# PathologyFoundation/plip

Measured on AMD Instinct MI355X. Metric: image+text pairs embedded/sec at 224px bs=256, higher is better.
Workload: dtype bf16; 1 GPU; full dual encoder (image tower + text tower + L2 normalise + logits_per_image), ViT-B/32, bs=256 pairs per GPU, 224px, 77 tokens, bf16 MFMA / fp32 accumulate (BASELINE.json configs[2]); the first 8 of the 12 text blocks on f16 MFMA operands (plipmi_config.text_f16_layers, the engine default); arch=ViT-B/32, per_gpu_batch=256, global_batch=256, parallelism=dp1, collective=none, streams=2, device=gfx950:sramecc+:xnack-:AMD Radeon Graphics

## Files before the change

### plip_amd/_lib.py

```python
from __future__ import annotations

import ctypes as C
import os
from typing import Optional

import torch

_HERE = os.path.dirname(os.path.abspath(__file__))
LIB_PATH = os.path.join(_HERE, "csrc", "libplipmi.so")

F32, BF16, F16 = 0, 1, 2
FLAG_SEPARATE_LAYERNORM, FLAG_DENSE_LAST_BLOCK, FLAG_PACK_CAPTIONS, FLAG_VALU_ATTENTION, FLAG_TEXT_TOWER_F16 = 1, 2, 4, 8, 16
FLAG_VISION_GELU, FLAG_TEXT_GELU = 32, 64
VISION, TEXT = 0, 1


class Config(C.Structure):
    _fields_ = [(n, C.c_int32) for n in (
        "struct_size", "image_size", "patch_size", "v_width", "v_layers", "v_heads", "v_mlp", "vocab_size",
        "context_length", "t_width", "t_layers", "t_heads", "t_mlp", "projection_dim")] + [
        ("layer_norm_eps", C.c_float), ("compute_dtype", C.c_int32), ("max_batch", C.c_int32), ("flags", C.c_int32),
        ("graph_batch", C.c_int32), ("text_f16_layers", C.c_int32), ("pass_batch", C.c_int32)]


_LAYER_FIELDS = ("ln1_w", "ln1_b", "q_w", "q_b", "k_w", "k_b", "v_w", "v_b", "o_w", "o_b",
                 "ln2_w", "ln2_b", "fc1_w", "fc1_b", "fc2_w", "fc2_b")


class LayerWeights(C.Structure):
    _fields_ = [(n, C.c_void_p) for n in _LAYER_FIELDS]


class Weights(C.Structure):
    _fields_ = [
        ("v_class_embedding", C.c_void_p), ("v_patch_weight", C.c_void_p), ("v_pos_embedding", C.c_void_p),
        ("v_pre_ln_w", C.c_void_p), ("v_pre_ln_b", C.c_void_p), ("v_post_ln_w", C.c_void_p),
        ("v_post_ln_b", C.c_void_p), ("visual_projection", C.c_void_p), ("v_layers", C.POINTER(LayerWeights)),
        ("t_token_embedding", C.c_void_p), ("t_pos_embedding", C.c_void_p), ("t_final_ln_w", C.c_void_p),
        ("t_final_ln_b", C.c_void_p), ("text_projection", C.c_void_p), ("t_layers", C.POINTER(LayerWeights)),
    ]


WEIGHT_KEYS = {
    "v_class_embedding": "vision_model.embeddings.class_embedding", "v_patch_weight": "vision_model.embeddings.patch_embedding.weight",
    "v_pos_embedding": "vision_model.embeddings.position_embedding.weight", "v_pre_ln_w": "vision_model.pre_layrnorm.weight",
    "v_pre_ln_b": "vision_model.pre_layrnorm.bias", "v_post_ln_w": "vision_model.post_layernorm.weight",
    "v_post_ln_b": "vision_model.post_layernorm.bias", "visual_projection": "visual_projection.weight",
    "t_token_embedding": "text_model.embeddings.token_embedding.weight", "t_pos_embedding": "text_model.embeddings.position_embedding.weight",
    "t_final_ln_w": "text_model.final_layer_norm.weight", "t_final_ln_b": "text_model.final_layer_norm.bias",
    "text_projection": "text_projection.weight"}
LAYER_KEYS = {"ln1": "layer_norm1", "ln2": "layer_norm2", "q": "self_attn.q_proj", "k": "self_attn.k_proj",
              "v": "self_attn.v_proj", "o": "self_attn.out_proj", "fc1": "mlp.fc1", "fc2": "mlp.fc2"}


class KernelStat(C.Structure):
    _fields_ = [("name", C.c_char * 96), ("calls", C.c_int64), ("total_ms", C.c_double),
                ("flops", C.c_double), ("bytes", C.c_double)]


PROBE_MAX_K = 64


class ProbeInfo(C.Structure):
    _fields_ = [("iterations", C.c_int32), ("evaluations", C.c_int32), ("converged", C.c_int32), ("reserved", C.c_int32),
                ("grad_norm", C.c_double), ("loss", C.c_double * PROBE_MAX_K)]


_vp, _i, _f = C.c_void_p, C.c_int, C.c_float
TEST_SYMBOLS = {
    "plipmi_debug_hidden": (_i, [_vp, _i, _i, _vp, _i, _vp, _vp]),
    "plipmi_gemm_nt": (_i, [_i, _i, _i, _i, _i, _i, _vp, _vp, _vp, _f, _vp, _vp]),
    "plipmi_gemm_variant_name": (C.c_char_p, [_i]),
    "plipmi_test_force_gemm_tile": (_i, [_i]),
    "plipmi_test_remap_gemm_tile": (_i, [_i, _i]),
    "plipmi_test_fused_qkv_attention": (_i, [_i]),
    "plipmi_test_patch_gather": (_i, [_i]),
    "plipmi_test_reset_hooks": (None, []),
    "plipmi_gemm_variant_built": (_i, [_i, _i]),
    "plipmi_recode_planes": (_i, [_vp, _vp, C.c_size_t, _i, _i, _i, _vp]),
    "plipmi_gemm_nt_ln": (_i, [_i, _i, _i, _i, _i, _i, _vp, _vp, _vp, _vp, _i, _f, _vp, _vp, _vp, _vp]),
    "plipmi_gemm_nt_ld": (_i, [_i, _i, _i, _i, _i, _i, _vp, _i, _vp, _i, _vp, _f, _vp, _vp]),
    "plipmi_gemm_nt_traced": (_i, [_i, _i, _i, _i, _i, _i, _vp, _vp, _vp, _f, _vp, _vp, _vp]),
    "plipmi_attention": (_i, [_i, _i, _vp, _vp, _i, _i, _i, _i, _vp, _vp]),
    "plipmi_qkv_attention": (_i, [_i, _vp, _vp, _vp, _vp, _i, _f, _vp, _i, _i, _i, _i, _vp, _vp, _vp]),
    "plipmi_resample_pos": (_i, [_vp, _vp, _i, _i, _i, _i, _vp]),
    "plipmi_probe_loss_grad": (_i, [_vp, _vp, _i, _i, _vp, _i, _vp, _vp, _f, _vp, _vp, _vp, _vp]),
    "plipmi_attention_probs": (_i, [_i, _vp, _vp, _i, _i, _i, _i, _vp, _vp]),
    "plipmi_attention_pooled_rows": (_i, [_i, _vp, _vp, _vp, _i, _i, _i, _i, _vp, _vp]),
    "plipmi_attention_rollout_step": (_i, [_i, _vp, _vp, _vp, _i, _i, _i, _i, _vp, _vp]),
    "plipmi_layernorm": (_i, [_vp, C.c_size_t, _vp, _vp, _vp, _i, _i, _i, _f, _vp]),
    "plipmi_layernorm_emit": (_i, [_i, _vp, _vp, _vp, _vp, _vp, _vp, _i, _i, _f, _vp]),
    "plipmi_fold_ln": (_i, [_i, _vp, _vp, _vp, _vp, _vp, _vp, _i, _i, _f, _vp]),
    "plipmi_text_embed_emit": (_i, [_i, _i, _vp, _vp, _vp, _vp, _vp, _vp, _i, _i, _i, _i, _i, _vp, _vp, _vp, _vp, _vp]),
    "plipmi_pool_rows": (_i, [_i, _vp, _i, _i, _i, _vp, _i, _vp, _vp, _f, _vp, _i, _i, _vp, _vp]),
    "plipmi_pool_gather": (_i, [_i, _vp, _vp, _vp, _i, _i, _i, _vp, _i, _vp, _vp, _vp, _vp]),
    "plipmi_head_gemm": (_i, [_vp, _vp, _vp, _i, _i, _i, _f, _vp]),
    "plipmi_resize_ragged_tables": (_i, [_i, _i, _i, _i, _i, _vp, _vp, _vp]),
    "plipmi_unfold_patches": (_i, [_i, _i, _vp, _vp, _i, _i, _i, _i, _i, _vp]),
    "plipmi_cls_rows": (_i, [_vp, _vp, _vp, _i, _i, _i, _vp]),
    "plipmi_gemm_patch": (_i, [_i, _i, _i, _i, _i, _vp, _i, _vp, _i, _vp, _i, _vp, _vp]),
    "plipmi_gemm_patch_gather": (_i, [_i, _vp, _vp, _vp, _vp, _vp, _i, _i, _i, _i, _i, _vp]),
    "plipmi_gemm_nt_ln_rows": (_i, [_i, _i, _i, _i, _i, _i, _vp, _vp, _vp, _vp, _i, _f, _vp, _vp, _vp, _vp, _vp]),
    "plipmi_attention_packed": (_i, [_i, _i, _vp, _vp, _i, _i, _i, _i, _vp, _vp, _vp]),
    "plipmi_gemm_nt_gelu": (_i, [_i, _i, _i, _i, _i, _i, _vp, _vp, _vp, _vp, _i, _f, _vp, _vp]),
}
SYMBOLS = {
    "plipmi_create": (_i, [C.POINTER(Config), C.POINTER(Weights), _vp, C.POINTER(_vp)]),
    "plipmi_destroy": (None, [_vp]),
    "plipmi_version": (_i, []),
    "plipmi_last_error": (C.c_char_p, []),
    "plipmi_device_name": (C.c_char_p, [_vp]),
    "plipmi_encode_image": (_i, [_vp, _vp, _i, _vp, _i, _vp]),
    "plipmi_encode_image_u8": (_i, [_vp, _vp, _i, _vp, _i, _vp]),
    "plipmi_encode_text": (_i, [_vp, _vp, _vp, _i, _i, _vp, _i, _vp]),
    "plipmi_check_async": (_i, [_vp]),
    "plipmi_set_latency_batch": (_i, [_vp, _i]),
    "plipmi_set_graph_batch": (_i, [_vp, _i]),
    "plipmi_get_pass_batch": (_i, [_vp]),
    "plipmi_clone": (_i, [_vp, C.POINTER(_vp)]),
    "plipmi_clone_resolution": (_i, [_vp, _i, _i, _i, C.POINTER(_vp)]),
    "plipmi_streams_overlap": (_i, [_vp, _vp, _vp, C.POINTER(_f)]),
    "plipmi_l2_normalize": (_i, [_vp, _vp, _i, _i, _vp]),
    "plipmi_logits": (_i, [_vp, _vp, _i, _vp, _i, _i, _f, _vp, _vp, _vp, _vp]),
    "plipmi_topk": (_i, [_vp, _vp, _i, _i, _i, _vp, _vp]),
    "plipmi_resize_crop_u8": (_i, [_vp, _vp, _i, _i, _i, _i, _vp, _vp, _i, _i, _vp, _vp, _i, _i, _i, _i, _vp, _vp, _vp]),
    "plipmi_resize_crop_u8_ragged": (_i, [_vp, _vp, C.c_size_t, _vp, _vp, _vp, _vp, _i, _i, _i, _i, _vp, C.c_size_t, _vp, _vp]),
    "plipmi_resize_ragged_workspace": (C.c_size_t, [_vp, _i, _i, _i]),
    "plipmi_similarity_topk": (_i, [_vp, _vp, _i, _vp, _i, _i, _i, _vp, _vp, _vp]),
    "plipmi_set_text_packing": (_i, [_vp, _i]),
    "plipmi_tower_shape": (_i, [_vp, _i, C.POINTER(C.c_int32)]),
    "plipmi_encode_tower_outputs": (_i, [_vp, _i, _vp, _vp, _i, _i, _vp, _vp, _vp, _vp, _vp]),
    "plipmi_encode_attention_summary": (_i, [_vp, _i, _vp, _vp, _i, _i, _vp, _vp, _vp, _vp]),
    "plipmi_probe_fit": (_i, [_vp, _vp, _i, _i, _vp, _i, _vp, _vp, _f, _i, _f, _vp, C.POINTER(ProbeInfo), _vp]),
    "plipmi_probe_predict": (_i, [_vp, _vp, _i, _i, _vp, _i, _vp, _vp, _vp]),
    "plipmi_profile_enable": (_i, [_vp, _i]),
    "plipmi_profile_read": (_i, [_vp, C.POINTER(KernelStat), _i, C.POINTER(_i)]),
}

_lib = None


def load():
    global _lib
    if _lib is not None:
        return _lib
    if not os.path.exists(LIB_PATH):
        raise RuntimeError(
            f"{LIB_PATH} is missing: the HIP engine is not built. Run `python -m plip_amd.build` "
            "(needs hipcc / ROCm). plip_amd has no fallback path.")
    try:
        lib = C.CDLL(LIB_PATH)
    except OSError as e:
        raise RuntimeError(f"cannot load {LIB_PATH}: {e}") from e
    for name, (res, args) in {**SYMBOLS, **TEST_SYMBOLS}.items():
        fn = getattr(lib, name)
        fn.restype = res
        fn.argtypes = args
    _lib = lib
    return lib
# ... 44 lines not shown
```

### plip_amd/csrc/engine.hip

```cpp
#include <stdio.h>
#include <time.h>

#include "handle_host.h"

namespace plipmi {

thread_local char g_err[512] = "";
int g_fuse_qkv_attention = 1;
int g_patch_gather = 1;
unsigned g_hook_epoch = 0;

int fail(int code, const char* fmt, ...) {
  va_list ap;
  va_start(ap, fmt);
  vsnprintf(g_err, sizeof(g_err), fmt, ap);
  va_end(ap);
  return code;
}

int check_async(plipmi_engine* e) {
  if (e->bad_id && *reinterpret_cast<volatile int*>(e->bad_id) != 0) {
    *reinterpret_cast<volatile int*>(e->bad_id) = 0;
    return fail(PLIPMI_ERR_TOKEN_ID, "an earlier plipmi_encode_text on this handle was given a token id outside [0, %d) "
                "(the reference's embedding lookup raises there, plip.py:68); its embeddings are invalid", e->cfg().vocab_size);
  }
  return PLIPMI_OK;
}
int check_batch(plipmi_engine* e, int B) {
  if (!e) return fail(PLIPMI_ERR_INVALID, "null handle");
  if (B < 0 || B > e->max_batch)
    return fail(PLIPMI_ERR_INVALID, "batch %d outside [0, max_batch=%d]", B, e->max_batch);
  return PLIPMI_OK;
}

}

using namespace plipmi;

namespace {

int pack_tower(const Model& m, const TowerModel& t, const plipmi_layer_weights* src, hipStream_t s) {
  const int D = t.D, F = t.F;
  const float qscale = 0.125f;
  for (int l = 0; l < t.L; ++l) {
    const int dt = t.layer_dtype(l);
    const plipmi_layer_weights& w = src[l];
    const LayerW& d = t.layers[l];
    char* wq = reinterpret_cast<char*>(d.wqkv);
    if (m.ln_fold) {
      HIP_TRY(launch_fold_ln(w.q_w, w.q_b, w.ln1_w, w.ln1_b, wq, d.bqkv, D, D, qscale, dt, s));
      HIP_TRY(launch_fold_ln(w.k_w, w.k_b, w.ln1_w, w.ln1_b, wq + (size_t)D * D * m.esz, d.bqkv + D, D, D, 1.f, dt, s));
      HIP_TRY(launch_fold_ln(w.v_w, w.v_b, w.ln1_w, w.ln1_b, wq + (size_t)2 * D * D * m.esz, d.bqkv + 2 * D, D, D, 1.f, dt, s));
      HIP_TRY(launch_fold_ln(w.fc1_w, w.fc1_b, w.ln2_w, w.ln2_b, d.w1, d.b1, F, D, 1.f, dt, s));
    } else {
      HIP_TRY(launch_convert(w.q_w, wq, dt, D, D, D, qscale, s));
      HIP_TRY(launch_convert(w.k_w, wq + (size_t)D * D * m.esz, dt, D, D, D, 1.f, s));
      HIP_TRY(launch_convert(w.v_w, wq + (size_t)2 * D * D * m.esz, dt, D, D, D, 1.f, s));
      HIP_TRY(launch_convert(w.fc1_w, d.w1, dt, F, D, D, 1.f, s));
      HIP_TRY(launch_scale_copy(w.q_b, d.bqkv, D, qscale, s));
      HIP_TRY(launch_scale_copy(w.k_b, d.bqkv + D, D, 1.f, s));
      HIP_TRY(launch_scale_copy(w.v_b, d.bqkv + 2 * D, D, 1.f, s));
      HIP_TRY(launch_scale_copy(w.fc1_b, d.b1, F, 1.f, s));
    }
    HIP_TRY(launch_convert(w.o_w, d.wo, dt, D, D, D, 1.f, s));
    HIP_TRY(launch_convert(w.fc2_w, d.w2, dt, D, F, F, 1.f, s));
    HIP_TRY(launch_scale_copy(w.o_b, d.bo, D, 1.f, s));
    HIP_TRY(launch_scale_copy(w.fc2_b, d.b2, D, 1.f, s));
    HIP_TRY(launch_scale_copy(w.ln1_w, d.ln1w, D, 1.f, s));
    HIP_TRY(launch_scale_copy(w.ln1_b, d.ln1b, D, 1.f, s));
    HIP_TRY(launch_scale_copy(w.ln2_w, d.ln2w, D, 1.f, s));
    HIP_TRY(launch_scale_copy(w.ln2_b, d.ln2b, D, 1.f, s));
  }
  return PLIPMI_OK;
}

int pack_model(const Model& m, const plipmi_weights* w, hipStream_t s) {
  const plipmi_config& g = m.cfg;
  const int Dv = g.v_width, Dt = g.t_width, P = g.projection_dim;
  HIP_TRY(launch_convert(w->v_patch_weight, m.patch_w, m.vis.dtype, Dv, 3 * g.patch_size * g.patch_size, m.kpad, 1.f, s));
  HIP_TRY(launch_scale_copy(w->v_class_embedding, m.cls, Dv, 1.f, s));
  HIP_TRY(launch_scale_copy(w->v_pos_embedding, m.vpos_native, m.native_tokens() * Dv, 1.f, s));
  HIP_TRY(launch_scale_copy(w->v_pre_ln_w, m.pre_w, Dv, 1.f, s));
  HIP_TRY(launch_scale_copy(w->v_pre_ln_b, m.pre_b, Dv, 1.f, s));
  HIP_TRY(launch_scale_copy(w->v_post_ln_w, m.vis.head_ln_w, Dv, 1.f, s));
  HIP_TRY(launch_scale_copy(w->v_post_ln_b, m.vis.head_ln_b, Dv, 1.f, s));
  HIP_TRY(launch_transpose(w->visual_projection, m.vis.proj_t, P, Dv, s));
  HIP_TRY(launch_scale_copy(w->visual_projection, m.vis.proj, P * Dv, 1.f, s));
  HIP_TRY(launch_scale_copy(w->text_projection, m.txt.proj, P * Dt, 1.f, s));
  HIP_TRY(hipMemcpyAsync(m.tok, w->t_token_embedding, (size_t)g.vocab_size * Dt * 4, hipMemcpyDeviceToDevice, s));
  HIP_TRY(launch_scale_copy(w->t_pos_embedding, m.tpos, g.context_length * Dt, 1.f, s));
  HIP_TRY(launch_scale_copy(w->t_final_ln_w, m.txt.head_ln_w, Dt, 1.f, s));
  HIP_TRY(launch_scale_copy(w->t_final_ln_b, m.txt.head_ln_b, Dt, 1.f, s));
  HIP_TRY(launch_transpose(w->text_projection, m.txt.proj_t, P, Dt, s));
  RUN(pack_tower(m, m.vis, w->v_layers, s));
  RUN(pack_tower(m, m.txt, w->t_layers, s));
  return PLIPMI_OK;
}

int alloc_workspace(plipmi_engine* e) {
  Carver sizing;
  carve_workspace(e, sizing);
  RUN(e->slab.reserve(align_up(sizing.off, 256), nullptr));
  Carver placing;
  placing.base = e->slab.data();
  carve_workspace(e, placing);
  if (e->bad_id_mem.reserve(sizeof(int), nullptr) == PLIPMI_OK) {
    e->bad_id = reinterpret_cast<int*>(e->bad_id_mem.data());
    *e->bad_id = 0;
  }
  return PLIPMI_OK;
}

int derive(plipmi_handle src, int max_batch, int height, int width, std::unique_ptr<plipmi_engine>* out) {
  auto e = std::make_unique<plipmi_engine>(src->model);
  shape_handle(e.get(), max_batch, height, width);
  e->graph_batch = std::min(src->graph_batch, e->graph_batch_cap);
  e->latency_batch = src->latency_batch;
  e->text_pack = src->text_pack;
  e->vpos = src->model->vpos_native;
  RUN(alloc_workspace(e.get()));
  *out = std::move(e);
  return PLIPMI_OK;
}

}

extern "C" {

int plipmi_version(void) { return PLIPMI_VERSION; }
const char* plipmi_last_error(void) { return g_err; }
const char* plipmi_device_name(plipmi_handle h) { return h ? h->model->devname : ""; }

int plipmi_create(const plipmi_config* cfg, const plipmi_weights* w, void* stream, plipmi_handle* out) {
  if (!cfg || !w || !out) return fail(PLIPMI_ERR_INVALID, "null argument");
  *out = nullptr;
  plipmi_config g;
  RUN(validate_config(cfg, &g));

  int dev = 0;
  hipDeviceProp_t prop;
  if (hipGetDevice(&dev) != hipSuccess || hipGetDeviceProperties(&prop, dev) != hipSuccess)
    return fail(PLIPMI_ERR_NODEVICE, "no HIP device visible (libplipmi needs an MI355X / gfx950 GPU)");
  if (strncmp(prop.gcnArchName, "gfx950", 6) != 0)
    return fail(PLIPMI_ERR_NODEVICE, "device %d is %s; libplipmi is built for gfx950 only", dev, prop.gcnArchName);

  auto m = std::make_shared<Model>();
  init_model(m.get(), g);
  snprintf(m->devname, sizeof(m->devname), "%s:%s", prop.gcnArchName, prop.name);
  Carver sizing;
  carve_weights(m.get(), sizing);
  RUN(m->slab.reserve(align_up(sizing.off, 256), nullptr));
  Carver placing;
  placing.base = m->slab.data();
  carve_weights(m.get(), placing);

  auto e = std::make_unique<plipmi_engine>(m);
  shape_handle(e.get(), g.max_batch, g.image_size, g.image_size);
  e->vpos = m->vpos_native;
  RUN(alloc_workspace(e.get()));
  RUN(pack_model(*m, w, reinterpret_cast<hipStream_t>(stream)));
  *out = e.release();
  return PLIPMI_OK;
}

int plipmi_clone(plipmi_handle src, plipmi_handle* out) {
  if (!src || !out) return fail(PLIPMI_ERR_INVALID, "null argument");
  *out = nullptr;
  std::unique_ptr<plipmi_engine> e;
  RUN(derive(src, src->max_batch, src->img_h, src->img_w, &e));
  e->vpos = src->vpos;
  e->vpos_own = src->vpos_own;
  *out = e.release();
  return PLIPMI_OK;
}

int plipmi_clone_resolution(plipmi_handle src, int height, int width, int max_batch, plipmi_handle* out) {
  if (!src || !out) return fail(PLIPMI_ERR_INVALID, "null argument");
  *out = nullptr;
  int B = 0;
  RUN(check_resolution(src, height, width, max_batch, &B));
  std::unique_ptr<plipmi_engine> e;
  RUN(derive(src, B, height, width, &e));
  const plipmi_config& g = src->cfg();
  const int n0 = g.image_size / g.patch_size;
  if (!(e->np == n0 * n0 && height == width)) {
    e->vpos_own = std::make_shared<Buffer>();
    RUN(e->vpos_own->reserve((size_t)e->vis.S * g.v_width * 4, nullptr));
    e->vpos = reinterpret_cast<float*>(e->vpos_own->data());
// ... 114 lines not shown
```

### plip_amd/csrc/gemm.h

```cpp
#pragma once
#include <hip/hip_runtime.h>

namespace plipmi {

enum Epilogue : int {
  EPI_BIAS = 0,
  EPI_BIAS_QGELU = 1,
  EPI_BIAS_RESID = 2,
  EPI_SCALE = 3,
  EPI_PATCH = 4,
  EPI_BIAS_LN = 5,
  EPI_QGELU_LN = 6,
  EPI_RESID_EMIT = 7,
  EPI_RESID_SPLIT = 8,
  EPI_BIAS_GELU = 9,
  EPI_GELU_LN = 10,
  EPI_COUNT = 11
};
constexpr bool epi_is_ln(int e) { return e == EPI_BIAS_LN || e == EPI_QGELU_LN || e == EPI_GELU_LN; }
constexpr bool epi_is_colwise(int e) { return e == EPI_BIAS || e == EPI_BIAS_QGELU || e == EPI_BIAS_GELU || epi_is_ln(e); }
constexpr bool epi_is_resid(int e) { return e == EPI_BIAS_RESID || e == EPI_RESID_EMIT || e == EPI_RESID_SPLIT; }
constexpr bool epi_emits_stats(int e) { return e == EPI_RESID_EMIT || e == EPI_RESID_SPLIT; }

struct GemmParams {
  const void* A;
  const void* W;
  void* C;
  const float* bias;
  int M, N, K;
  int lda, ldw, ldc;
  float alpha;
  int np;
  const float* ln_stats = nullptr;
  int ln_ns = 0;
  float ln_inv_d = 0.f, ln_eps = 0.f;
  void* xb_out = nullptr;
  float* st_out = nullptr;
  void* lo_io = nullptr;
  int planes_other = 0;
  const float* pix = nullptr;
  int img_h = 0, img_w = 0, patch_log2 = 0;
  const unsigned char* tiles = nullptr;
  const int* m_dev = nullptr;
  int gw = 0;
  unsigned long long* trace = nullptr;
};

struct GemmVariant {
  const char* name;
  int bm, bn, threads;
};
int gemm_num_variants();
int gemm_num_cus();
const GemmVariant& gemm_variant(int v);
int gemm_launch(int dtype, int epi, int variant, const GemmParams& p, hipStream_t stream, const char** kernel_name);
int gemm_default_variant(int dtype, int M, int N, int K);
bool gemm_variant_is_built(int dtype, int variant);
bool gemm_skinny_supports(int epi, int M, int N, int K);
int gemm_launch_skinny(int dtype, int epi, const GemmParams& p, hipStream_t stream, const char** kernel_name);
bool gemm_force_tile(int variant);
bool gemm_remap_tile(int from, int to);
void gemm_reset_overrides();
bool gemm_gather_supports(int dtype, int B, int img_h, int img_w, int patch, int N);
int gemm_launch_gather(int dtype, const GemmParams& p, hipStream_t stream, const char** kernel_name);

}
```

### plip_amd/csrc/gemm_skinny.hip

```cpp
#include "gemm_skinny_kernel.h"

namespace plipmi {

bool gemm_skinny_supports(int epi, int M, int N, int K) {
  const bool epi_ok = epi == EPI_BIAS || epi == EPI_BIAS_QGELU || epi == EPI_BIAS_RESID || epi == EPI_BIAS_LN ||
                      epi == EPI_QGELU_LN || epi == EPI_RESID_EMIT || epi == EPI_RESID_SPLIT || epi == EPI_PATCH ||
                      epi == EPI_BIAS_GELU || epi == EPI_GELU_LN;
  return epi_ok && M > 0 && N % SK_BN == 0 && K % 256 == 0;
}

template <typename T>
static int launch_skinny_epi(int epi, const GemmParams& p, hipStream_t s) {
  switch (epi) {
    case EPI_BIAS: return launch_skinny<T, EPI_BIAS>(p, s);
    case EPI_BIAS_QGELU: return launch_skinny<T, EPI_BIAS_QGELU>(p, s);
    case EPI_BIAS_RESID: return launch_skinny<T, EPI_BIAS_RESID>(p, s);
    case EPI_BIAS_LN: return launch_skinny<T, EPI_BIAS_LN>(p, s);
    case EPI_QGELU_LN: return launch_skinny<T, EPI_QGELU_LN>(p, s);
    case EPI_RESID_EMIT: return launch_skinny<T, EPI_RESID_EMIT>(p, s);
    case EPI_RESID_SPLIT: return launch_skinny<T, EPI_RESID_SPLIT>(p, s);
    case EPI_PATCH: return launch_skinny<T, EPI_PATCH>(p, s);
    default: return (int)hipErrorInvalidValue;
  }
}

int gemm_launch_skinny(int dtype, int epi, const GemmParams& p, hipStream_t s, const char** kernel_name) {
  if (p.M <= 0) return 0;
  if ((dtype != 1 && dtype != 2) || !gemm_skinny_supports(epi, p.M, p.N, p.K) || p.lda % 8 || p.ldw % 8) return (int)hipErrorInvalidValue;
  static const char* names[2][EPI_COUNT] = {
      {"gemm_skinny<bf16,32x64_splitk,bias>", "gemm_skinny<bf16,32x64_splitk,bias_qgelu>", "gemm_skinny<bf16,32x64_splitk,bias_resid>",
       nullptr, "gemm_skinny<bf16,32x64_splitk,patch>", "gemm_skinny<bf16,32x64_splitk,ln_bias>", "gemm_skinny<bf16,32x64_splitk,ln_qgelu>",
       "gemm_skinny<bf16,32x64_splitk,resid_emit>", "gemm_skinny<bf16,32x64_splitk,resid_split>",
       "gemm_skinny<bf16,32x64_splitk,bias_gelu>", "gemm_skinny<bf16,32x64_splitk,ln_gelu>"},
      {"gemm_skinny<f16,32x64_splitk,bias>", "gemm_skinny<f16,32x64_splitk,bias_qgelu>", "gemm_skinny<f16,32x64_splitk,bias_resid>",
       nullptr, "gemm_skinny<f16,32x64_splitk,patch>", "gemm_skinny<f16,32x64_splitk,ln_bias>", "gemm_skinny<f16,32x64_splitk,ln_qgelu>",
       "gemm_skinny<f16,32x64_splitk,resid_emit>", "gemm_skinny<f16,32x64_splitk,resid_split>",
       "gemm_skinny<f16,32x64_splitk,bias_gelu>", "gemm_skinny<f16,32x64_splitk,ln_gelu>"}};
  if (kernel_name) *kernel_name = names[dtype - 1][epi];
  if (epi == EPI_BIAS_GELU || epi == EPI_GELU_LN) return gemm_launch_skinny_gelu(dtype, epi, p, s);
  return with_half(dtype, [&](auto tag) { return launch_skinny_epi<decltype(tag)>(epi, p, s); });
}

}
```

### plip_amd/csrc/gemm_skinny_kernel.h

```cpp
#pragma once
#include "dispatch.h"
#include "gemm.h"
#include "gemm_lds.h"

namespace plipmi {

namespace {

constexpr int SK_BM = 32, SK_BN = 64, SK_PITCH = 68;

template <typename T, int EPI, int NW, int NB>
__global__ __launch_bounds__(64 * NW) void gemm_skinny_kernel(const GemmParams p) {
  using X8 = typename half_traits<T>::x8;
  __shared__ __attribute__((aligned(16))) float part[NW][SK_BM][SK_PITCH];
  __shared__ float rs_s[SK_BM];
  const int tid = threadIdx.x, lane = tid & 63;
  const int wave = __builtin_amdgcn_readfirstlane(tid >> 6);
  const int lrow = lane & 31, hi = lane >> 5;
  const int n0 = blockIdx.x * SK_BN, m0 = blockIdx.y * SK_BM;
  const int kw = p.K / NW;
  const int mr = m0 + lrow < p.M ? m0 + lrow : p.M - 1;
  const T* ap = reinterpret_cast<const T*>(p.A) + (size_t)mr * p.lda + wave * kw + 32 * hi;
  const T* w0 = reinterpret_cast<const T*>(p.W) + (size_t)(n0 + lrow) * p.ldw + wave * kw + 32 * hi;
  const T* w1 = w0 + (size_t)32 * p.ldw;

  if constexpr (epi_is_ln(EPI)) {
    if (tid < SK_BM) {
      const int r = m0 + tid < p.M ? m0 + tid : p.M - 1;
      float mu, rs;
      ln_combine(p.ln_stats + (size_t)r * p.ln_ns * 2, p.ln_ns, p.ln_inv_d, p.ln_eps, mu, rs);
      rs_s[tid] = rs;
    }
  }

  f32x16 acc0, acc1;
#pragma unroll
  for (int e = 0; e < 16; ++e) { acc0[e] = 0.f; acc1[e] = 0.f; }
#pragma unroll 1
  for (int kk = 0; kk < kw; kk += 64 * NB) {
    u32x4 xa[NB][4], wa[NB][4], wb[NB][4];
#pragma unroll
    for (int b = 0; b < NB; ++b)
#pragma unroll
      for (int t = 0; t < 4; ++t) {
        xa[b][t] = *reinterpret_cast<const u32x4*>(ap + kk + 64 * b + 8 * t);
        wa[b][t] = *reinterpret_cast<const u32x4*>(w0 + kk + 64 * b + 8 * t);
        wb[b][t] = *reinterpret_cast<const u32x4*>(w1 + kk + 64 * b + 8 * t);
      }
    __builtin_amdgcn_sched_barrier(0);
#pragma unroll
    for (int b = 0; b < NB; ++b)
#pragma unroll
      for (int t = 0; t < 4; ++t) {
        acc0 = half_traits<T>::mfma32(__builtin_bit_cast(X8, wa[b][t]), __builtin_bit_cast(X8, xa[b][t]), acc0);
        acc1 = half_traits<T>::mfma32(__builtin_bit_cast(X8, wb[b][t]), __builtin_bit_cast(X8, xa[b][t]), acc1);
      }
  }
#pragma unroll
  for (int q = 0; q < 4; ++q) {
    *reinterpret_cast<f32x4*>(&part[wave][lrow][8 * q + 4 * hi]) = f32x4{acc0[4 * q], acc0[4 * q + 1], acc0[4 * q + 2], acc0[4 * q + 3]};
    *reinterpret_cast<f32x4*>(&part[wave][lrow][32 + 8 * q + 4 * hi]) = f32x4{acc1[4 * q], acc1[4 * q + 1], acc1[4 * q + 2], acc1[4 * q + 3]};
  }
  __syncthreads();
  if (tid >= 256) return;
  const int r = tid >> 3, c8 = (tid & 7) * 8;
  float v[8];
#pragma unroll
  for (int h = 0; h < 2; ++h) {
    f32x4 sum4[NW / 4];
#pragma unroll
    for (int g = 0; g < NW / 4; ++g) {
      const f32x4 a = *reinterpret_cast<const f32x4*>(&part[4 * g + 0][r][c8 + 4 * h]), b = *reinterpret_cast<const f32x4*>(&part[4 * g + 1][r][c8 + 4 * h]);
      const f32x4 c = *reinterpret_cast<const f32x4*>(&part[4 * g + 2][r][c8 + 4 * h]), d = *reinterpret_cast<const f32x4*>(&part[4 * g + 3][r][c8 + 4 * h]);
#pragma unroll
      for (int e = 0; e < 4; ++e) sum4[g][e] = (a[e] + b[e]) + (c[e] + d[e]);
    }
#pragma unroll
    for (int e = 0; e < 4; ++e) v[4 * h + e] = NW == 8 ? sum4[0][e] + sum4[NW / 4 - 1][e] : sum4[0][e];
  }
  const int m = m0 + r, n = n0 + c8;
  const bool in_range = m < p.M;
  const float4 b0 = *reinterpret_cast<const float4*>(p.bias + n), b1 = *reinterpret_cast<const float4*>(p.bias + n + 4);
  const float bias[8] = {b0.x, b0.y, b0.z, b0.w, b1.x, b1.y, b1.z, b1.w};
  if constexpr (epi_is_colwise(EPI)) {
    const float rs = epi_is_ln(EPI) ? rs_s[r] : 1.0f;
    X8 o;
#pragma unroll
    for (int e = 0; e < 8; ++e) {
      float y = fmaf(rs, v[e], bias[e]);
      if constexpr (EPI == EPI_BIAS_QGELU || EPI == EPI_QGELU_LN) y = quick_gelu<false>(y);
      if constexpr (EPI == EPI_BIAS_GELU || EPI == EPI_GELU_LN) y = erf_gelu<false>(y);
      o[e] = from_f32<T>(y);
    }
    if (in_range) *reinterpret_cast<X8*>(reinterpret_cast<T*>(p.C) + (size_t)m * p.ldc + n) = o;
  } else if constexpr (EPI == EPI_PATCH) {
    const int mm = in_range ? m : p.M - 1;
    const int img = mm / p.np, pp = mm - img * p.np;
    const float4 p0 = *reinterpret_cast<const float4*>(p.bias + (size_t)(1 + pp) * p.N + n), p1 = *reinterpret_cast<const float4*>(p.bias + (size_t)(1 + pp) * p.N + n + 4);
    float* crow = reinterpret_cast<float*>(p.C) + ((size_t)img * (p.np + 1) + 1 + pp) * p.ldc + n;
    if (in_range) {
      *reinterpret_cast<float4*>(crow) = make_float4(v[0] + p0.x, v[1] + p0.y, v[2] + p0.z, v[3] + p0.w);
      *reinterpret_cast<float4*>(crow + 4) = make_float4(v[4] + p1.x, v[5] + p1.y, v[6] + p1.z, v[7] + p1.w);
    }
  } else if constexpr (EPI == EPI_RESID_SPLIT) {
    const size_t mr = (size_t)(in_range ? m : p.M - 1);
    const size_t off = mr * p.ldc + n;
    const size_t loff = lo_plane_off(mr, (unsigned)n, (unsigned)p.ldc);
    const u32x4 h = *reinterpret_cast<const u32x4*>(reinterpret_cast<const unsigned short*>(p.xb_out) + off);
    const uint2 l = *reinterpret_cast<const uint2*>(reinterpret_cast<const unsigned char*>(p.lo_io) + loff);
    float o[8], s = 0.f;
#pragma unroll
    for (int e = 0; e < 4; ++e) {
      o[2 * e] = join_f32<T>(h[e] & 0xffffu, sbyte(e < 2 ? l.x : l.y, (2 * e) & 3));
      o[2 * e + 1] = join_f32<T>(h[e] >> 16, sbyte(e < 2 ? l.x : l.y, (2 * e + 1) & 3));
    }
#pragma unroll
    for (int e = 0; e < 8; ++e) o[e] = (o[e] + bias[e]) + v[e];
    s = ((o[0] + o[1]) + (o[2] + o[3])) + ((o[4] + o[5]) + (o[6] + o[7]));
    const float ssum = row8_sum(s);
    const float mj = ssum * (1.0f / kLnSlice);
    float q = 0.f;
#pragma unroll
    for (int e = 0; e < 8; ++e) { const float d = o[e] - mj; q = fmaf(d, d, q); }
    const float m2 = row8_sum(q);
    if (in_range) {
      u32x4 ho;
      unsigned lb[8];
#pragma unroll
      for (int e = 0; e < 4; ++e) {
        unsigned ha, hb;
        split_f32<T>(o[2 * e], ha, lb[2 * e]);
        split_f32<T>(o[2 * e + 1], hb, lb[2 * e + 1]);
        ho[e] = ha | (hb << 16);
      }
      *reinterpret_cast<u32x4*>(reinterpret_cast<unsigned short*>(p.xb_out) + off) = ho;
      *reinterpret_cast<uint2*>(reinterpret_cast<unsigned char*>(p.lo_io) + loff) =
          make_uint2(lb[0] | (lb[1] << 8) | (lb[2] << 16) | (lb[3] << 24), lb[4] | (lb[5] << 8) | (lb[6] << 16) | (lb[7] << 24));
      if ((tid & 7) == 0) *reinterpret_cast<float2*>(p.st_out + ((size_t)m * (p.N / kLnSlice) + n0 / kLnSlice) * 2) = make_float2(ssum, m2);
    }
  } else {
    static_assert(epi_is_resid(EPI), "skinny epilogues: bias / QuickGELU / GELU (optionally LayerNorm-folded), patch rows and the residual forms");
    float* crow = reinterpret_cast<float*>(p.C) + (size_t)(in_range ? m : p.M - 1) * p.ldc + n;
    const float4 x0 = *reinterpret_cast<const float4*>(crow), x1 = *reinterpret_cast<const float4*>(crow + 4);
    const float xo[8] = {x0.x, x0.y, x0.z, x0.w, x1.x, x1.y, x1.z, x1.w};
    float o[8], s = 0.f;
#pragma unroll
    for (int e = 0; e < 8; ++e) { o[e] = xo[e] + (v[e] + bias[e]); s += o[e]; }
    if (in_range) {
      *reinterpret_cast<float4*>(crow) = make_float4(o[0], o[1], o[2], o[3]);
      *reinterpret_cast<float4*>(crow + 4) = make_float4(o[4], o[5], o[6], o[7]);
    }
    if constexpr (EPI == EPI_RESID_EMIT) {
      const float ssum = row8_sum(s);
      const float mj = ssum * (1.0f / kLnSlice);
      float q = 0.f;
#pragma unroll
      for (int e = 0; e < 8; ++e) { const float d = o[e] - mj; q += d * d; }
      const float m2 = row8_sum(q);
      if (in_range) {
        X8 ob;
#pragma unroll
        for (int e = 0; e < 8; ++e) ob[e] = from_f32<T>(o[e]);
        *reinterpret_cast<X8*>(reinterpret_cast<T*>(p.xb_out) + (size_t)m * p.ldc + n) = ob;
        if ((tid & 7) == 0) *reinterpret_cast<float2*>(p.st_out + ((size_t)m * (p.N / kLnSlice) + n0 / kLnSlice) * 2) = make_float2(ssum, m2);
      }
    }
  }
}

template <typename T, int EPI, int NW, int NB>
int launch_skinny_nb(const GemmParams& p, hipStream_t s) {
  const dim3 grid(p.N / SK_BN, (p.M + SK_BM - 1) / SK_BM);
  hipLaunchKernelGGL((gemm_skinny_kernel<T, EPI, NW, NB>), grid, dim3(64 * NW), 0, s, p);
  return (int)hipGetLastError();
}
template <typename T, int EPI>
int launch_skinny(const GemmParams& p, hipStream_t s) {
  const int blocks = p.K / 64;
  if (blocks % 8 == 0) {
    const int nb = blocks / 8;
    if (nb % 3 == 0) return launch_skinny_nb<T, EPI, 8, 3>(p, s);
    if (nb % 2 == 0) return launch_skinny_nb<T, EPI, 8, 2>(p, s);
    return launch_skinny_nb<T, EPI, 8, 1>(p, s);
  }
  const int nb = blocks / 4;
  if (nb % 3 == 0) return launch_skinny_nb<T, EPI, 4, 3>(p, s);
  return launch_skinny_nb<T, EPI, 4, 1>(p, s);
}

}

int gemm_launch_skinny_gelu(int dtype, int epi, const GemmParams& p, hipStream_t s);

}
```

### plip_amd/csrc/handle.h

```cpp
#pragma once
#include <stdarg.h>
#include <stdint.h>
#include <string.h>

#include <map>
#include <memory>
#include <string>
#include <tuple>
#include <type_traits>
#include <vector>

#include "../../include/plipmi.h"
#include "../../include/plipmi_test.h"
#include "gemm.h"
#include "kernels.h"

namespace plipmi {

extern thread_local char g_err[512];
extern int g_fuse_qkv_attention;
extern int g_patch_gather;
extern unsigned g_hook_epoch;

int fail(int code, const char* fmt, ...);
// ... 73 lines not shown
    if (stream_) hipStreamDestroy(stream_);
  }
  void clear() {
    for (auto& kv : entries_) if (kv.second.exec) hipGraphExecDestroy(kv.second.exec);
    entries_.clear();
  }
  GraphEntry& at(const Key& k) {
    if (epoch_ != g_hook_epoch) {
      clear();
      epoch_ = g_hook_epoch;
    }
    return entries_[k];
  }
  hipError_t capture_stream(hipStream_t* out) {
    const hipError_t e = stream_ ? hipSuccess : hipStreamCreateWithFlags(&stream_, hipStreamNonBlocking);
    *out = stream_;
    return e;
  }

 private:
  std::map<Key, GraphEntry> entries_;
  unsigned epoch_ = 0;
  hipStream_t stream_ = nullptr;
};

struct ProfRec {
  const char* name;
  hipEvent_t t0, t1;
  double flops, bytes;
};
struct Profile {
  bool on = false;
  std::vector<ProfRec> recs;
  std::vector<hipEvent_t> pool;
  Profile() = default;
  Profile(const Profile&) = delete;
  Profile& operator=(const Profile&) = delete;
  ~Profile() {
    for (ProfRec& r : recs) { hipEventDestroy(r.t0); hipEventDestroy(r.t1); }
    for (hipEvent_t ev : pool) hipEventDestroy(ev);
  }
};

struct LayerW {
  void *wqkv, *wo, *w1, *w2;
  float *bqkv, *bo, *b1, *b2, *ln1w, *ln1b, *ln2w, *ln2b;
};
struct TowerModel {
  int D = 0, F = 0, L = 0, H = 0;
  int dtype = 0;
  int lead_f16 = 0;
  int layer_dtype(int l) const { return l < lead_f16 ? PLIPMI_F16 : dtype; }
  bool gelu = false;
  int fc1_epi(bool ln_folded) const { return ln_folded ? (gelu ? EPI_GELU_LN : EPI_QGELU_LN) : (gelu ? EPI_BIAS_GELU : EPI_BIAS_QGELU); }
  std::vector<LayerW> layers;
  float *head_ln_w = nullptr, *head_ln_b = nullptr, *proj = nullptr, *proj_t = nullptr;
};
struct Model {
  plipmi_config cfg;
  int dtype = 0;
  size_t esz = 4;
  bool ln_fold = false;
  bool pooled_last = false;
  int kpad = 0;
  TowerModel vis, txt;
  void* patch_w = nullptr;
  float *cls = nullptr, *vpos_native = nullptr , *pre_w = nullptr, *pre_b = nullptr;
  float *tok = nullptr, *tpos = nullptr;
  Buffer slab;
  char devname[128] = "";
  bool half() const { return dtype != PLIPMI_F32; }
  int native_tokens() const { return (cfg.image_size / cfg.patch_size) * (cfg.image_size / cfg.patch_size) + 1; }
};

struct Tower {
  const TowerModel* m = nullptr;
  int S = 0;
  float* x = nullptr;
  void *h = nullptr, *qkv = nullptr, *att = nullptr, *mlp = nullptr;
  float* st = nullptr;
  void* lo = nullptr;
  int *cu = nullptr, *rowmap = nullptr, *mdev = nullptr;
  float* xp = nullptr; void *attp = nullptr, *hp = nullptr, *mlpp = nullptr; float* stp = nullptr;
  float* pooled = nullptr;
};

}

struct plipmi_engine {
  const std::shared_ptr<const plipmi::Model> model;
  int max_batch = 0;
  int img_h = 0, img_w = 0, gh = 0, gw = 0, np = 0;
  float* vpos = nullptr;
  std::shared_ptr<plipmi::Buffer> vpos_own;
  int pass_batch = 0;
  int graph_batch = 0, graph_batch_cap = 0;
  int latency_batch = 0;
  bool text_pack = false;
  int attn_impl = 0, attn_impl_vis = 0, attn_impl_txt = 0;
  plipmi::Buffer slab;
  plipmi::Tower vis, txt;
  void* patches = nullptr;
  void* g_vin = nullptr;
  int64_t* g_tin = nullptr;
  int64_t* g_tmask = nullptr;
  float *g_vout = nullptr, *g_tout = nullptr;
  plipmi::GraphCache graphs;
  plipmi::Buffer bad_id_mem{plipmi::Buffer::kPinnedMapped};
  int* bad_id = nullptr;
  plipmi::Buffer sim_ws;
  plipmi::Buffer summary_ws;
  plipmi::Buffer probe_ws, probe_host{plipmi::Buffer::kPinned};
  plipmi::Profile prof;

  explicit plipmi_engine(std::shared_ptr<const plipmi::Model> m) : model(std::move(m)) {
    vis.m = &model->vis;
    txt.m = &model->txt;
    txt.S = model->cfg.context_length;
  }
  const plipmi_config& cfg() const { return model->cfg; }
  bool half() const { return model->half(); }
};
static_assert(!std::is_copy_constructible_v<plipmi_engine> && !std::is_copy_assignable_v<plipmi_engine>,
              "a handle owns its workspace, graphs and scratch: a clone is constructed from the model, never copied");

namespace plipmi {

struct Scope {
  Profile& p;
  hipStream_t s;
  bool on;
  ProfRec r;
  Scope(plipmi_engine* e, hipStream_t s_, const char* name, double flops, double bytes) : p(e->prof), s(s_), on(e->prof.on) {
    if (!on) return;
    r.name = name; r.flops = flops; r.bytes = bytes;
    r.t0 = take(); r.t1 = take();
    hipEventRecord(r.t0, s);
  }
  void rename(const char* name) { r.name = name; }
  ~Scope() {
    if (!on) return;
    hipEventRecord(r.t1, s);
    p.recs.push_back(r);
  }
  hipEvent_t take() {
    if (!p.pool.empty()) { hipEvent_t ev = p.pool.back(); p.pool.pop_back(); return ev; }
    hipEvent_t ev; hipEventCreate(&ev); return ev;
  }
};

inline GemmParams make_params(const void* A, const void* W, void* C, const float* bias, int M, int N, int K, int lda, int ldw, int ldc) {
  GemmParams p;
  p.A = A; p.W = W; p.C = C; p.bias = bias;
  p.M = M; p.N = N; p.K = K; p.lda = lda; p.ldw = ldw; p.ldc = ldc;
  p.alpha = 1.f; p.np = 1;
  return p;
}

int check_batch(plipmi_engine* e, int B);
int check_async(plipmi_engine* e);

}
```

### plip_amd/csrc/towers.hip

```cpp
#include "handle_host.h"

using namespace plipmi;

namespace {

struct LnArgs {
  const float* stats = nullptr; int ns = 0; float inv_d = 0.f, eps = 0.f;
  void* xb_out = nullptr; float* st_out = nullptr; void* lo_io = nullptr;
  int planes_other = 0;
};
struct Taps {
  float* hidden = nullptr;
  float* probs = nullptr;
  float* pooled_rows = nullptr;
  float* rollout[2] = {nullptr, nullptr};
  const int* row_idx = nullptr;
  bool attention() const { return probs || pooled_rows || rollout[0]; }
};

struct Forward {
  plipmi_engine* e;
  const Model& md;
  const TowerModel& m;
  Tower& t;
  const bool vision;
  const int B;
  hipStream_t s;
  const int causal;
  const int64_t* key_mask;
  bool small = false;
  bool packed = false;
  int cur, planes;
  const Taps* taps = nullptr;

  enum Regime { kEncode, kEveryToken };
  Forward(plipmi_engine* e_, int tower, int B_, const int64_t* mask, hipStream_t s_, Regime r, bool may_pack)
      : e(e_), md(*e_->model), m(tower == PLIPMI_VISION ? md.vis : md.txt), t(tower == PLIPMI_VISION ? e_->vis : e_->txt),
        vision(tower == PLIPMI_VISION), B(B_), s(s_), causal(vision ? 0 : 1), key_mask(mask), cur(m.layer_dtype(0)), planes(cur) {
    small = r == kEncode && e->half() && B <= e->latency_batch;
    packed = may_pack && !vision && e->text_pack && md.ln_fold && md.pooled_last && e->attn_impl_txt == 1 && t.S <= 128;
  }
  int M() const { return B * t.S; }
  int attn_impl() const { return vision ? e->attn_impl_vis : e->attn_impl_txt; }
  const int* cu() const { return packed ? t.cu : nullptr; }
  const int* m_dev() const { return packed ? t.mdev : nullptr; }
  LnArgs ln_use(const float* stats) const {
    LnArgs a; a.stats = stats; a.ns = m.D / kLnSlice; a.inv_d = 1.0f / (float)m.D; a.eps = md.cfg.layer_norm_eps;
    return a;
  }
};

const char* name_with_role(const char* name, const char* role) {
  static thread_local std::map<std::pair<const char*, const char*>, std::string> cache;
  std::string& v = cache[std::make_pair(name, role)];
  if (v.empty()) v = std::string(name) + "|" + role;
  return v.c_str();
}

int run_gemm(Forward& f, int epi, const void* A, const void* W, void* C, const float* bias, int M, int N, int K,
             int ldc, int np, const char* role, const LnArgs* ln = nullptr, const int* m_dev = nullptr) {
  plipmi_engine* e = f.e;
  GemmParams p = make_params(A, W, C, bias, M, N, K, K, K, ldc);
  p.m_dev = m_dev; p.np = np;
  if (ln) {
    p.ln_stats = ln->stats; p.ln_ns = ln->ns; p.ln_inv_d = ln->inv_d; p.ln_eps = ln->eps;
    p.xb_out = ln->xb_out; p.st_out = ln->st_out; p.lo_io = ln->lo_io; p.planes_other = ln->planes_other;
  }
  bool skinny = role[0] == '~';
  if (skinny) ++role;
  skinny = skinny || (f.small && !m_dev);
  const char* name = "gemm_nt";
  const double out_bytes = epi_is_colwise(epi) ? (double)M * N * f.md.esz
                           : (double)M * N * (epi == EPI_RESID_SPLIT ? 6.0 : epi_is_resid(epi) ? 8.0 : 4.0) + (epi == EPI_RESID_EMIT ? (double)M * N * 2.0 : 0.0);
  Scope sc(e, f.s, name, 2.0 * M * N * (double)K, ((double)M * K + (double)N * K) * f.md.esz + out_bytes);
  const int rc = (skinny && e->half() && gemm_skinny_supports(epi, M, N, K))
                     ? gemm_launch_skinny(f.cur, epi, p, f.s, &name)
                     : gemm_launch(f.cur, epi, -1, p, f.s, &name);
  if (e->prof.on) sc.rename(name_with_role(name, role));
  if (rc != 0) return fail(PLIPMI_ERR_HIP, "gemm launch (%s, M=%d N=%d K=%d) failed: %s", name, M, N, K,
                           hipGetErrorString((hipError_t)rc));
  return PLIPMI_OK;
}

int enter_block(Forward& f, int l) {
  f.cur = f.m.layer_dtype(l);
  if (f.md.ln_fold && f.planes != f.cur) {
    Scope sc(f.e, f.s, "recode_planes", 0, (double)f.M() * f.m.D * 6);
    HIP_TRY(launch_recode_planes(f.t.h, f.t.lo, (size_t)f.M(), f.m.D, f.planes, f.cur, f.s));
    f.planes = f.cur;
  }
  return PLIPMI_OK;
}

int run_attention(Forward& f, int tap) {
  const Tower& t = f.t;
  const int H = f.m.H, S = t.S, B = f.B;
  const Taps* taps = tap >= 0 ? f.taps : nullptr;
  if (taps && taps->probs) {
    Scope sc(f.e, f.s, "attention_probs", 2.0 * B * H * (double)S * S * 64, (double)B * H * S * S * 4);
    HIP_TRY(launch_attention_probs(t.qkv, taps->probs + (size_t)tap * B * H * S * S, f.cur, B, S, H, f.causal, f.key_mask, f.s));
  }
  if (taps && taps->pooled_rows && !taps->rollout[0]) {
    Scope sc(f.e, f.s, "attention_pooled_rows", 2.0 * B * H * (double)S * 64, (double)B * H * S * (4 + 2.0 * 64 * f.md.esz));
    HIP_TRY(launch_attention_pooled_rows(t.qkv, taps->row_idx, taps->pooled_rows + (size_t)tap * B * H * S, f.cur, B, S, H, f.causal,
                                         f.key_mask, f.s));
  }
  if (taps && taps->rollout[0]) {
    Scope sc(f.e, f.s, "attention_rollout_step", 2.0 * B * H * (double)S * S * 64 + 2.0 * B * (double)S * S * S,
             (double)B * S * (2.0 * H * 64 * f.md.esz + 8.0 * S));
    HIP_TRY(launch_attention_rollout_step(t.qkv, tap == 0 ? nullptr : taps->rollout[(tap - 1) & 1], taps->rollout[tap & 1], f.cur, B, S, H,
                                          f.causal, f.key_mask, f.s, taps->row_idx,
                                          taps->pooled_rows ? taps->pooled_rows + (size_t)tap * B * H * S : nullptr));
  }
  const int impl = f.attn_impl();
  Scope sc(f.e, f.s, impl ? "attention_mfma" : "attention_valu", 4.0 * B * H * (double)S * S * 64, (double)f.M() * 4 * f.m.D * f.md.esz);
  HIP_TRY(launch_attention(t.qkv, t.att, f.cur, B, S, H, f.causal, f.key_mask, impl, f.s, f.cu()));
  return PLIPMI_OK;
}

int run_qkv_attention(Forward& f, const LayerW& w, const LnArgs& use, int tap = -1) {
  Tower& t = f.t;
  const int M = f.M(), D = f.m.D, H = f.m.H, B = f.B;
  if (tap < 0 && g_fuse_qkv_attention && f.attn_impl() == 1 && !f.packed && !f.small && qkv_attention_supports(f.cur, B, t.S, H, D) &&
      (g_fuse_qkv_attention == 2 || qkv_attention_pays(B, H, gemm_num_cus()))) {
    Scope sc(f.e, f.s, "qkv_attention", 2.0 * M * 3.0 * D * (double)D + 4.0 * B * H * (double)t.S * t.S * 64, ((double)M * D * 2 + 3.0 * D * D) * f.md.esz);
    HIP_TRY(launch_qkv_attention(f.cur, t.h, w.wqkv, w.bqkv, use.stats, use.inv_d, use.eps, t.att, B, t.S, H, f.causal, f.key_mask, f.s));
    return PLIPMI_OK;
  }
  RUN(run_gemm(f, EPI_BIAS_LN, t.h, w.wqkv, t.qkv, w.bqkv, M, 3 * D, D, 3 * D, 0, "qkv", &use, f.m_dev()));
  return run_attention(f, tap);
}

int run_layers(Forward& f, int n_layers, bool more_follow = false) {
  plipmi_engine* e = f.e;
  Tower& t = f.t;
  const int M = f.M(), D = f.m.D, F = f.m.F;
  hipStream_t s = f.s;
  auto tap_of = [&](int l) { return f.taps && f.taps->attention() ? l : -1; };
  auto hidden_of = [&](int l) -> float* { return f.taps && f.taps->hidden ? f.taps->hidden + (size_t)(l + 1) * M * D : nullptr; };
  const float eps = f.md.cfg.layer_norm_eps;
  const int* md = f.m_dev();
  if (f.md.ln_fold) {
    const LnArgs use = f.ln_use(t.st);
    LnArgs emit; emit.xb_out = t.h; emit.st_out = t.st; emit.lo_io = t.lo;
    for (int l = 0; l < n_layers; ++l) {
      const LayerW& w = f.m.layers[l];
      RUN(enter_block(f, l));
      RUN(run_qkv_attention(f, w, use, tap_of(l)));
      RUN(run_gemm(f, EPI_RESID_SPLIT, t.att, w.wo, nullptr, w.bo, M, D, D, D, 0, "out_proj", &emit, md));
      RUN(run_gemm(f, f.m.fc1_epi(true), t.h, w.w1, t.mlp, w.b1, M, F, D, F, 0, "fc1", &use, md));
      const int next_dt = l + 1 < f.m.L ? f.m.layer_dtype(l + 1) : f.cur;
      LnArgs emit2 = emit;
// ... 326 lines not shown
```

Measured before the change: 60540 pairs/s.

## Split skinny GEMM K across two workgroups with atomic-ticket reduction

When the skinny GEMM grid has at most half as many tiles as there are CUs, the 8-wave K split is launched as two 4-wave workgroups along grid z. Each writes its partial tile to a global scratch slab, and the second to arrive (decided by an atomic ticket per tile) adds the other partial and runs the epilogue. This aims to fill more CUs on the small-M pooled last-block GEMMs, at the cost of an extra global round trip, fences, and a per-tower workspace with counters.

```diff
diff --git a/plip_amd/_lib.py b/plip_amd/_lib.py
--- a/plip_amd/_lib.py
+++ b/plip_amd/_lib.py
@@ -75,6 +75,8 @@
     "plipmi_test_remap_gemm_tile": (_i, [_i, _i]),
     "plipmi_test_fused_qkv_attention": (_i, [_i]),
     "plipmi_test_patch_gather": (_i, [_i]),
+    "plipmi_test_skinny_kslices": (_i, [_i, _vp, _i]),
+    "plipmi_skinny_kslices": (_i, [_i, _i, _i]),
     "plipmi_test_reset_hooks": (None, []),
     "plipmi_gemm_variant_built": (_i, [_i, _i]),
     "plipmi_recode_planes": (_i, [_vp, _vp, C.c_size_t, _i, _i, _i, _vp]),
diff --git a/plip_amd/csrc/engine.hip b/plip_amd/csrc/engine.hip
--- a/plip_amd/csrc/engine.hip
+++ b/plip_amd/csrc/engine.hip
@@ -104,6 +104,15 @@
   Carver placing;
   placing.base = e->slab.data();
   carve_workspace(e, placing);
+  if (e->model->pooled_last) {
+    const size_t cnt = kSkinnyKsTiles * sizeof(unsigned), part = (size_t)kSkinnyKsTiles * 2 * 32 * 64 * sizeof(float);
+    RUN(e->ks_mem.reserve(2 * (cnt + part), nullptr));
+    char* base = e->ks_mem.data();
+    e->vis.ks_cnt = reinterpret_cast<unsigned*>(base);               e->txt.ks_cnt = reinterpret_cast<unsigned*>(base + cnt);
+    e->vis.ks_part = reinterpret_cast<float*>(base + 2 * cnt);       e->txt.ks_part = reinterpret_cast<float*>(base + 2 * cnt + part);
+    HIP_TRY(hipMemset(base, 0, 2 * cnt));
+    HIP_TRY(hipStreamSynchronize(nullptr));
+  }
   if (e->bad_id_mem.reserve(sizeof(int), nullptr) == PLIPMI_OK) {
     e->bad_id = reinterpret_cast<int*>(e->bad_id_mem.data());
     *e->bad_id = 0;
diff --git a/plip_amd/csrc/gemm.h b/plip_amd/csrc/gemm.h
--- a/plip_amd/csrc/gemm.h
+++ b/plip_amd/csrc/gemm.h
@@ -42,6 +42,9 @@
   int img_h = 0, img_w = 0, patch_log2 = 0;
   const unsigned char* tiles = nullptr;
   const int* m_dev = nullptr;
+  unsigned* ks_cnt = nullptr;
+  float* ks_part = nullptr;
+  int ks_tiles = 0;
   int gw = 0;
   unsigned long long* trace = nullptr;
 };
@@ -58,6 +61,9 @@
 bool gemm_variant_is_built(int dtype, int variant);
 bool gemm_skinny_supports(int epi, int M, int N, int K);
 int gemm_launch_skinny(int dtype, int epi, const GemmParams& p, hipStream_t stream, const char** kernel_name);
+constexpr int kSkinnyKsTiles = 256;
+int gemm_skinny_kslices(const GemmParams& p);
+bool gemm_skinny_force_kslices(int ks);
 bool gemm_force_tile(int variant);
 bool gemm_remap_tile(int from, int to);
 void gemm_reset_overrides();
diff --git a/plip_amd/csrc/gemm_skinny.hip b/plip_amd/csrc/gemm_skinny.hip
--- a/plip_amd/csrc/gemm_skinny.hip
+++ b/plip_amd/csrc/gemm_skinny.hip
@@ -8,6 +8,14 @@
                       epi == EPI_BIAS_GELU || epi == EPI_GELU_LN;
   return epi_ok && M > 0 && N % SK_BN == 0 && K % 256 == 0;
 }
+
+int g_skinny_ks = 0;
+bool gemm_skinny_force_kslices(int ks) {
+  if (ks < 0 || ks > 2) return false;
+  g_skinny_ks = ks;
+  return true;
+}
+int gemm_skinny_kslices(const GemmParams& p) { return skinny_kslices(p, g_skinny_ks, gemm_num_cus()); }
 
 template <typename T>
 static int launch_skinny_epi(int epi, const GemmParams& p, hipStream_t s) {
diff --git a/plip_amd/csrc/gemm_skinny_kernel.h b/plip_amd/csrc/gemm_skinny_kernel.h
--- a/plip_amd/csrc/gemm_skinny_kernel.h
+++ b/plip_amd/csrc/gemm_skinny_kernel.h
@@ -5,12 +5,15 @@
 
 namespace plipmi {
 
+extern int g_skinny_ks;
+
 namespace {
 
 constexpr int SK_BM = 32, SK_BN = 64, SK_PITCH = 68;
 
-template <typename T, int EPI, int NW, int NB>
+template <typename T, int EPI, int NW, int NB, int KS>
 __global__ __launch_bounds__(64 * NW) void gemm_skinny_kernel(const GemmParams p) {
+  static_assert(KS == 1 || (KS == 2 && NW == 4), "two K slices are the 8-wave split run as two 4-wave workgroups");
   using X8 = typename half_traits<T>::x8;
   __shared__ __attribute__((aligned(16))) float part[NW][SK_BM][SK_PITCH];
   __shared__ float rs_s[SK_BM];
@@ -18,10 +21,11 @@
   const int wave = __builtin_amdgcn_readfirstlane(tid >> 6);
   const int lrow = lane & 31, hi = lane >> 5;
   const int n0 = blockIdx.x * SK_BN, m0 = blockIdx.y * SK_BM;
-  const int kw = p.K / NW;
+  const int kw = p.K / (NW * KS);
+  const int kwave = KS == 1 ? wave : (int)blockIdx.z * NW + wave;
   const int mr = m0 + lrow < p.M ? m0 + lrow : p.M - 1;
-  const T* ap = reinterpret_cast<const T*>(p.A) + (size_t)mr * p.lda + wave * kw + 32 * hi;
-  const T* w0 = reinterpret_cast<const T*>(p.W) + (size_t)(n0 + lrow) * p.ldw + wave * kw + 32 * hi;
+  const T* ap = reinterpret_cast<const T*>(p.A) + (size_t)mr * p.lda + kwave * kw + 32 * hi;
+  const T* w0 = reinterpret_cast<const T*>(p.W) + (size_t)(n0 + lrow) * p.ldw + kwave * kw + 32 * hi;
   const T* w1 = w0 + (size_t)32 * p.ldw;
 
   if constexpr (epi_is_ln(EPI)) {
@@ -77,6 +81,33 @@
     }
 #pragma unroll
     for (int e = 0; e < 4; ++e) v[4 * h + e] = NW == 8 ? sum4[0][e] + sum4[NW / 4 - 1][e] : sum4[0][e];
+  }
+  if constexpr (KS == 2) {
+    const int slice = blockIdx.z, tile = blockIdx.y * gridDim.x + blockIdx.x;
+    float* slab = p.ks_part + (size_t)tile * (2 * SK_BM * SK_BN);
+    float* mine = slab + slice * (SK_BM * SK_BN) + tid * 8;
+    *reinterpret_cast<f32x4*>(mine) = f32x4{v[0], v[1], v[2], v[3]};
+    *reinterpret_cast<f32x4*>(mine + 4) = f32x4{v[4], v[5], v[6], v[7]};
+    asm volatile("s_waitcnt vmcnt(0)" ::: "memory");
+    __syncthreads();
+    if (tid == 0) {
+      __builtin_amdgcn_fence(__ATOMIC_RELEASE, "agent");
+      asm volatile("s_waitcnt vmcnt(0)" ::: "memory");
+      const unsigned ticket = __hip_atomic_fetch_add(p.ks_cnt + tile, 1u, __ATOMIC_RELAXED, __HIP_MEMORY_SCOPE_AGENT);
+      if (ticket == 1) {
+        __hip_atomic_store(p.ks_cnt + tile, 0u, __ATOMIC_RELAXED, __HIP_MEMORY_SCOPE_AGENT);
+        __builtin_amdgcn_fence(__ATOMIC_ACQUIRE, "agent");
+        asm volatile("s_waitcnt vmcnt(0)" ::: "memory");
+      }
+      part[0][0][SK_BN] = ticket == 1 ? 1.0f : 0.0f;
+    }
+    __syncthreads();
+    if (part[0][0][SK_BN] == 0.0f) return;
+    const float* other = slab + (1 - slice) * (SK_BM * SK_BN) + tid * 8;
+    const f32x4 o0 = *reinterpret_cast<const f32x4*>(other), o1 = *reinterpret_cast<const f32x4*>(other + 4);
+    const float ov[8] = {o0[0], o0[1], o0[2], o0[3], o1[0], o1[1], o1[2], o1[3]};
+#pragma unroll
+    for (int e = 0; e < 8; ++e) v[e] = slice == 0 ? v[e] + ov[e] : ov[e] + v[e];
   }
   const int m = m0 + r, n = n0 + c8;
   const bool in_range = m < p.M;
@@ -169,19 +200,31 @@
 }
 
 template <typename T, int EPI, int NW, int NB>
-int launch_skinny_nb(const GemmParams& p, hipStream_t s) {
-  const dim3 grid(p.N / SK_BN, (p.M + SK_BM - 1) / SK_BM);
-  hipLaunchKernelGGL((gemm_skinny_kernel<T, EPI, NW, NB>), grid, dim3(64 * NW), 0, s, p);
+int launch_skinny_nb(const GemmParams& p, hipStream_t s, int ks = 1) {
+  const dim3 grid(p.N / SK_BN, (p.M + SK_BM - 1) / SK_BM, ks);
+  if constexpr (NW == 8) {
+    if (ks == 2) {
+      hipLaunchKernelGGL((gemm_skinny_kernel<T, EPI, 4, NB, 2>), grid, dim3(64 * 4), 0, s, p);
+      return (int)hipGetLastError();
+    }
+  }
+  hipLaunchKernelGGL((gemm_skinny_kernel<T, EPI, NW, NB, 1>), grid, dim3(64 * NW), 0, s, p);
   return (int)hipGetLastError();
+}
+inline int skinny_kslices(const GemmParams& p, int force, int num_cus) {
+  const long long tiles = (long long)(p.N / SK_BN) * ((p.M + SK_BM - 1) / SK_BM);
+  if ((p.K / 64) % 8 != 0 || !p.ks_cnt || !p.ks_part || tiles > p.ks_tiles || force == 1) return 1;
+  return force == 2 || tiles * 2 <= num_cus ? 2 : 1;
 }
 template <typename T, int EPI>
 int launch_skinny(const GemmParams& p, hipStream_t s) {
   const int blocks = p.K / 64;
   if (blocks % 8 == 0) {
     const int nb = blocks / 8;
-    if (nb % 3 == 0) return launch_skinny_nb<T, EPI, 8, 3>(p, s);
-    if (nb % 2 == 0) return launch_skinny_nb<T, EPI, 8, 2>(p, s);
-    return launch_skinny_nb<T, EPI, 8, 1>(p, s);
+    const int ks = skinny_kslices(p, g_skinny_ks, gemm_num_cus());
+    if (nb % 3 == 0) return launch_skinny_nb<T, EPI, 8, 3>(p, s, ks);
+    if (nb % 2 == 0) return launch_skinny_nb<T, EPI, 8, 2>(p, s, ks);
+    return launch_skinny_nb<T, EPI, 8, 1>(p, s, ks);
   }
   const int nb = blocks / 4;
   if (nb % 3 == 0) return launch_skinny_nb<T, EPI, 4, 3>(p, s);
diff --git a/plip_amd/csrc/handle.h b/plip_amd/csrc/handle.h
--- a/plip_amd/csrc/handle.h
+++ b/plip_amd/csrc/handle.h
@@ -179,6 +179,7 @@
   void* lo = nullptr;
   int *cu = nullptr, *rowmap = nullptr, *mdev = nullptr;
   float* xp = nullptr; void *attp = nullptr, *hp = nullptr, *mlpp = nullptr; float* stp = nullptr;
+  unsigned* ks_cnt = nullptr; float* ks_part = nullptr;
   float* pooled = nullptr;
 };
 
@@ -205,6 +206,7 @@
   plipmi::GraphCache graphs;
   plipmi::Buffer bad_id_mem{plipmi::Buffer::kPinnedMapped};
   int* bad_id = nullptr;
+  plipmi::Buffer ks_mem;
   plipmi::Buffer sim_ws;
   plipmi::Buffer summary_ws;
   plipmi::Buffer probe_ws, probe_host{plipmi::Buffer::kPinned};
diff --git a/plip_amd/csrc/towers.hip b/plip_amd/csrc/towers.hip
--- a/plip_amd/csrc/towers.hip
+++ b/plip_amd/csrc/towers.hip
@@ -67,7 +67,10 @@
     p.xb_out = ln->xb_out; p.st_out = ln->st_out; p.lo_io = ln->lo_io; p.planes_other = ln->planes_other;
   }
   bool skinny = role[0] == '~';
-  if (skinny) ++role;
+  if (skinny) {
+    ++role;
+    p.ks_cnt = f.t.ks_cnt; p.ks_part = f.t.ks_part; p.ks_tiles = kSkinnyKsTiles;
+  }
   skinny = skinny || (f.small && !m_dev);
   const char* name = "gemm_nt";
   const double out_bytes = epi_is_colwise(epi) ? (double)M * N * f.md.esz
```

Result: no change. 60530 pairs/s, median of 2 (-0.0%).
